# PRBonn/OverlapNet

Measured on AMD Instinct MI355X. Metric: scan-pairs/s (64x900 range images), higher is better.
Workload: dtype f32 (scaled 3-term fp16 split on the fp16 MFMA: 22 significand bits per operand, fp32 accumulate)

## Files before the change

overlapnet_amd/csrc/c3_dense.hip:

```cpp
#include "ovn_internal.h"

typedef _Float16 f16x8 __attribute__((ext_vector_type(8)));
typedef _Float16 f16x4 __attribute__((ext_vector_type(4)));

namespace {

struct ArithF16 {
  typedef _Float16 elem;
  typedef f16x8 v8;
  typedef f16x4 v4;
  static __device__ __forceinline__ f32x4 mfma(v8 a, v8 b, f32x4 c) { return __builtin_amdgcn_mfma_f32_16x16x32_f16(a, b, c, 0, 0, 0); }
};

constexpr int G = OVN_G;
constexpr int OW = OVN_O3_HW;
constexpr int CI = OVN_C2_OUT;
constexpr int CO = OVN_C3_OUT;
constexpr int NBAND = 3;
constexpr int MAX_ROWS = 8;
constexpr int MAX_MT = (MAX_ROWS * OW + 15) / 16;
constexpr int IN_PIX_MAX = (MAX_ROWS + 2) * G;
constexpr int PLANE = IN_PIX_MAX * 8 + 8;
constexpr int NPL = CI / 8;
constexpr size_t LDS_BYTES = 2 * (size_t)NPL * PLANE * sizeof(_Float16) + 64;
constexpr int NW = 8;

__device__ __forceinline__ int band_start(int b) { return b == 0 ? 0 : (b == 1 ? 8 : 15); }
__device__ __forceinline__ int band_rows(int b) { return b == 0 ? 8 : 7; }

constexpr int MT_SPLIT = 6;
template <class A, int NWV, int MSPLIT>
__global__ __launch_bounds__(64 * NWV) void c3_dense_kernel(const float* __restrict__ o2, const typename A::elem* __restrict__ wp,
                                                           const float* __restrict__ b3, const float* __restrict__ wd,
                                                           const unsigned* __restrict__ o2max, float sw3,
                                                           float* __restrict__ partial, float* __restrict__ o3,
                                                           unsigned* __restrict__ arrived, const float* __restrict__ bd,
                                                           float* __restrict__ overlap, float* __restrict__ logit) {
  typedef typename A::elem elem_t;
  typedef typename A::v8 v8_t;
  typedef typename A::v4 v4_t;
  extern __shared__ __attribute__((aligned(16))) unsigned char smem[];
  elem_t* ih = reinterpret_cast<elem_t*>(smem);
  elem_t* il = ih + NPL * PLANE;
  float* red = reinterpret_cast<float*>(il + NPL * PLANE);

  constexpr int HALVES = NW / NWV;
  constexpr int MTW = MSPLIT == 1 ? MAX_MT : MT_SPLIT;
  const int sub = blockIdx.x % (HALVES * MSPLIT);
  const int unit = blockIdx.x / (HALVES * MSPLIT), half = sub % HALVES, mh = sub / HALVES;
  const int mt0 = MT_SPLIT * mh;
  const int pair = unit / NBAND;
  const int band = unit - pair * NBAND;
  const int r0 = band_start(band);
  const int nrows = band_rows(band);
  const int npix = nrows * OW;
  const int nmt = (npix + 15) >> 4;
  const int tid = threadIdx.x;
  const int lane = tid & 63;
  const int wave_l = tid >> 6;
  const int wave = wave_l + NWV * half;
  const int lrow = lane & 15;
  const int g = lane >> 4;

  const elem_t* wsrc = wp + ((size_t)(2 * wave) * 2) * 512 + lane * 8;
  v8_t bq[3][4];
#define C3_LOAD_B(DST, KC)                                                                  \
  {                                                                                         \
    const elem_t* q = wsrc + (size_t)(KC) * (16 * 2 * 512);                                 \
    DST[0] = *reinterpret_cast<const v8_t*>(q);                                           \
    DST[1] = *reinterpret_cast<const v8_t*>(q + 512);                                     \
    DST[2] = *reinterpret_cast<const v8_t*>(q + 1024);                                    \
    DST[3] = *reinterpret_cast<const v8_t*>(q + 1536);                                    \
  }
  C3_LOAD_B(bq[0], 0)
  C3_LOAD_B(bq[1], 1)
  const float s2 = ovn_pow2_scale_for(__uint_as_float(o2max[pair]));
  const float inv = 1.0f / (s2 * sw3);
  {
    const float* src = o2 + ((long long)pair * G + r0) * G * CI;
    const int n4 = (nrows + 2) * G * CI / 4;
    constexpr int PER_THREAD = (MAX_ROWS + 2) * G * CI / 4 / (64 * NWV);
    static_assert(PER_THREAD * 64 * NWV == (MAX_ROWS + 2) * G * CI / 4, "patch does not divide over the threads");
    f32x4 v[PER_THREAD];
#pragma unroll
    for (int k = 0; k < PER_THREAD; ++k) {
      const int i = tid + k * (64 * NWV);
      v[k] = (i < n4) ? *reinterpret_cast<const f32x4*>(src + 4 * i) : (f32x4){0.f, 0.f, 0.f, 0.f};
    }
#pragma unroll
    for (int k = 0; k < PER_THREAD; ++k) {
      const int i = tid + k * (64 * NWV);
      if (i < n4) {
        const int pix = i / (CI / 4);
        const int c = 4 * (i - pix * (CI / 4));
        v4_t h, l;
#pragma unroll
        for (int e = 0; e < 4; ++e) {
          const float x = v[k][e] * s2;
          h[e] = (elem_t)x;
          l[e] = (elem_t)(x - (float)h[e]);
        }
        const int o = (c >> 3) * PLANE + pix * 8 + (c & 7);
        *reinterpret_cast<v4_t*>(ih + o) = h;
        *reinterpret_cast<v4_t*>(il + o) = l;
      }
    }
  }

  int abase[MTW];
#pragma unroll
  for (int mt = 0; mt < MTW; ++mt) {
    int p = 16 * (mt0 + mt) + lrow;
    if (p >= npix) p = npix - 1;
    const int oy = p / OW;
    const int ox = p - oy * OW;
    abase[mt] = g * PLANE + (oy * G + ox) * 8;
  }

  f32x4 acc[MTW][2];
#pragma unroll
  for (int mt = 0; mt < MTW; ++mt) {
    acc[mt][0] = (f32x4){0.f, 0.f, 0.f, 0.f};
    acc[mt][1] = (f32x4){0.f, 0.f, 0.f, 0.f};
  }

#define C3_MFMA2(M0, M1, A0H, A0L, A1H, A1L, SRC)                                                  \
  acc[M0][0] = A::mfma(A0H, SRC[0], acc[M0][0]);          \
  acc[M0][1] = A::mfma(A0H, SRC[2], acc[M0][1]);          \
  acc[M1][0] = A::mfma(A1H, SRC[0], acc[M1][0]);          \
  acc[M1][1] = A::mfma(A1H, SRC[2], acc[M1][1]);          \
  acc[M0][0] = A::mfma(A0L, SRC[0], acc[M0][0]);          \
  acc[M0][1] = A::mfma(A0L, SRC[2], acc[M0][1]);          \
  acc[M1][0] = A::mfma(A1L, SRC[0], acc[M1][0]);          \
  acc[M1][1] = A::mfma(A1L, SRC[2], acc[M1][1]);          \
  acc[M0][0] = A::mfma(A0H, SRC[1], acc[M0][0]);          \
  acc[M0][1] = A::mfma(A0H, SRC[3], acc[M0][1]);          \
  acc[M1][0] = A::mfma(A1H, SRC[1], acc[M1][0]);          \
  acc[M1][1] = A::mfma(A1H, SRC[3], acc[M1][1]);
#define C3_READ_A(BUF, SLOT, MT)                                                            \
  fh[BUF][SLOT] = *reinterpret_cast<const v8_t*>(ih + abase[MT] + toff);                  \
  fl[BUF][SLOT] = *reinterpret_cast<const v8_t*>(il + abase[MT] + toff);
#define C3_STEP(SRC, KC)                                                                    \
  {                                                                                         \
    const int tap = (KC) >> 2;                                                              \
    const int ky = tap / 3;                                                                 \
    const int toff = (ky * G + (tap - 3 * ky)) * 8 + 4 * PLANE * ((KC) & 3);                \
    v8_t fh[2][2], fl[2][2];                                                              \
    C3_READ_A(0, 0, 0)                                                                      \
    C3_READ_A(0, 1, 1)                                                                      \
    _Pragma("unroll") for (int q = 0; q < MTW / 2; ++q) {                                \
      const int cb = q & 1, nb = cb ^ 1;                                                    \
      if (q + 1 < MTW / 2) {                                                             \
        C3_READ_A(nb, 0, 2 * q + 2)                                                         \
        C3_READ_A(nb, 1, 2 * q + 3)                                                         \
      } else if (MTW % 2 == 1 && nmt == MAX_MT) {                                                           \
        C3_READ_A(nb, 0, MTW - 1)                                                        \
      }                                                                                     \
      __builtin_amdgcn_sched_barrier(0);   \
      C3_MFMA2(2 * q, 2 * q + 1, fh[cb][0], fl[cb][0], fh[cb][1], fl[cb][1], SRC)           \
      __builtin_amdgcn_sched_barrier(0);                                                    \
    }                                                                                       \
    if (MTW % 2 == 1 && nmt == MAX_MT) {                               \
      const v8_t ah = fh[(MTW / 2) & 1][0], al = fl[(MTW / 2) & 1][0];              \
      acc[MTW - 1][0] = A::mfma(ah, SRC[0], acc[MTW - 1][0]); \
      acc[MTW - 1][1] = A::mfma(ah, SRC[2], acc[MTW - 1][1]); \
      acc[MTW - 1][0] = A::mfma(al, SRC[0], acc[MTW - 1][0]); \
      acc[MTW - 1][1] = A::mfma(al, SRC[2], acc[MTW - 1][1]); \
      acc[MTW - 1][0] = A::mfma(ah, SRC[1], acc[MTW - 1][0]); \
      acc[MTW - 1][1] = A::mfma(ah, SRC[3], acc[MTW - 1][1]); \
    }                                                                                       \
  }
  __syncthreads();
#pragma unroll 1
  for (int kc = 0; kc < 36; kc += 3) {
    C3_LOAD_B(bq[2], kc + 2)
    C3_STEP(bq[0], kc)
    if (kc + 3 < 36) C3_LOAD_B(bq[0], kc + 3)
    C3_STEP(bq[1], kc + 1)
    if (kc + 4 < 36) C3_LOAD_B(bq[1], kc + 4)
    C3_STEP(bq[2], kc + 2)
  }
#undef C3_LOAD_B
#undef C3_STEP
#undef C3_MFMA2
#undef C3_READ_A

  float s[2] = {0.f, 0.f};
#pragma unroll
  for (int nt = 0; nt < 2; ++nt) {
    const int n = 32 * wave + 16 * nt + lrow;
    const float bv = b3[n];
#pragma unroll
    for (int mt = 0; mt < MTW; ++mt) {
#pragma unroll
      for (int r = 0; r < 4; ++r) {
        const int p = 16 * (mt0 + mt) + 4 * g + r;
        if (p < npix) {
          const float v = fmaxf(fmaf(acc[mt][nt][r], inv, bv), 0.0f);
          const long long fi = (long long)(r0 * OW + p) * CO + n;
          s[(MSPLIT == 1 && mt >= MT_SPLIT) ? 1 : 0] += v * wd[fi];
          if (o3) o3[(long long)pair * OVN_DENSE_IN + fi] = v;
        }
      }
    }
  }
#pragma unroll
  for (int off = 32; off > 0; off >>= 1) {
    s[0] += __shfl_down(s[0], off, 64);
    if (MSPLIT == 1) s[1] += __shfl_down(s[1], off, 64);
  }
  if (lane == 0) {
    red[wave_l] = s[0];
    if (MSPLIT == 1) red[NW + wave_l] = s[1];
  }
  __syncthreads();
  if (tid == 0) {
    float* dst = partial + ((size_t)pair * NBAND + band) * 4;
    if (NWV == NW) {
      dst[0] = (red[0] + red[1]) + (red[2] + red[3]);
      dst[1] = (red[NW + 0] + red[NW + 1]) + (red[NW + 2] + red[NW + 3]);
      dst[2] = (red[4] + red[5]) + (red[6] + red[7]);
      dst[3] = (red[NW + 4] + red[NW + 5]) + (red[NW + 6] + red[NW + 7]);
    } else {
      dst[2 * half + mh] = (red[0] + red[1]) + (red[2] + red[3]);
    }
    if (overlap != nullptr) {
      constexpr unsigned PARTS = NBAND * HALVES * MSPLIT;
      __threadfence();
      const unsigned prev = atomicAdd(arrived + pair, 1u);
      if (prev == PARTS - 1) {
        __threadfence();
        const float* q = partial + (size_t)pair * OVN_DENSE_PARTIALS;
        float z = 0.f;
#pragma unroll
        for (int b = 0; b < NBAND; ++b) {
          const float q0 = __hip_atomic_load(q + 4 * b, __ATOMIC_RELAXED, __HIP_MEMORY_SCOPE_AGENT);
          const float q1 = __hip_atomic_load(q + 4 * b + 1, __ATOMIC_RELAXED, __HIP_MEMORY_SCOPE_AGENT);
          const float q2 = __hip_atomic_load(q + 4 * b + 2, __ATOMIC_RELAXED, __HIP_MEMORY_SCOPE_AGENT);
          const float q3 = __hip_atomic_load(q + 4 * b + 3, __ATOMIC_RELAXED, __HIP_MEMORY_SCOPE_AGENT);
          const float zb = (q0 + q1) + (q2 + q3);
          z = b == 0 ? zb : z + zb;
        }
        z += bd[0];
        if (logit) logit[pair] = z;
        overlap[pair] = 1.0f / (1.0f + expf(-z));
        __hip_atomic_store(arrived + pair, 0u, __ATOMIC_RELAXED, __HIP_MEMORY_SCOPE_AGENT);
      }
    }
  }
}

__global__ __launch_bounds__(256) void dense_finish_kernel(const float* __restrict__ partial, const float* __restrict__ bd, int n,
                                                           float* __restrict__ overlap, float* __restrict__ logit) {
  const int p = blockIdx.x * 256 + threadIdx.x;
  if (p >= n) return;
  const float* q = partial + (size_t)p * OVN_DENSE_PARTIALS;
  float z = 0.f;
#pragma unroll
  for (int b = 0; b < NBAND; ++b) {
    const float zb = (q[4 * b] + q[4 * b + 1]) + (q[4 * b + 2] + q[4 * b + 3]);
    z = b == 0 ? zb : z + zb;
  }
  z += bd[0];
  if (logit) logit[p] = z;
  overlap[p] = 1.0f / (1.0f + expf(-z));
}

}

int ovn_c3_dense_forward(const ovn_ctx* ctx, const float* o2, const unsigned* o2max, int n, float* partial, float* o3,
                         unsigned* arrived, float* overlap, float* logit, hipStream_t stream) {
  OVN_REQUIRE(o2max != nullptr, OVN_ERR_ARG, "ovn_c3_dense_forward: the per-pair maxima of o2 are required");
  OVN_REQUIRE(overlap == nullptr || arrived != nullptr, OVN_ERR_ARG, "ovn_c3_dense_forward: arrival counters missing");
  int rc;
  if (n <= 21) {
    rc = ovn_allow_dynamic_lds(reinterpret_cast<const void*>(c3_dense_kernel<ArithF16, 4, 2>), LDS_BYTES);
    if (rc) return rc;
    hipLaunchKernelGGL((c3_dense_kernel<ArithF16, 4, 2>), dim3(4 * NBAND * n), dim3(64 * 4), LDS_BYTES, stream, o2,
                       reinterpret_cast<const _Float16*>(ctx->head.c3.wp_h), ctx->head.c3.bias, ctx->head.wd, o2max, ctx->head.c3.sw_h, partial, o3, arrived,
                       ctx->head.bd, overlap, logit);
  } else {
    rc = ovn_allow_dynamic_lds(reinterpret_cast<const void*>(c3_dense_kernel<ArithF16, NW, 1>), LDS_BYTES);
    if (rc) return rc;
    hipLaunchKernelGGL((c3_dense_kernel<ArithF16, NW, 1>), dim3(NBAND * n), dim3(64 * NW), LDS_BYTES, stream, o2,
                       reinterpret_cast<const _Float16*>(ctx->head.c3.wp_h), ctx->head.c3.bias, ctx->head.wd, o2max, ctx->head.c3.sw_h, partial, o3,
                       (unsigned*)nullptr, ctx->head.bd, (float*)nullptr, (float*)nullptr);
    if (overlap != nullptr)
      hipLaunchKernelGGL(dense_finish_kernel, dim3((n + 255) / 256), dim3(256), 0, stream, partial, ctx->head.bd, n, overlap, logit);
  }
  OVN_HIP_CHECK(hipGetLastError());
  return OVN_OK;
}
```

overlapnet_amd/csrc/delta_head_f16x3.hip:

```cpp
#include <math.h>
#include <stdlib.h>

#include <initializer_list>
#include <type_traits>

#include "ovn_internal.h"
#include "delta_a2.h"

typedef _Float16 f16x8 __attribute__((ext_vector_type(8)));
typedef _Float16 f16x4 __attribute__((ext_vector_type(4)));
typedef _Float16 f16x2 __attribute__((ext_vector_type(2)));
typedef __bf16 bf16x8 __attribute__((ext_vector_type(8)));

namespace {

constexpr int FW = OVN_FEAT_W;
constexpr int FC = OVN_FEAT_C;
constexpr int S = OVN_S;
constexpr int G = OVN_G;
constexpr int O1 = OVN_C1_OUT;
constexpr int O2 = OVN_C2_OUT;
constexpr int K1 = S * FC;
constexpr int K2 = S * O1;
constexpr int STEP_BYTES = 8192;
// ... 422 lines not shown
  if (packed && tid >= 64 && tid < 96) {
    const int k = tid - 64;
    if (k >= n_last) chan_s[32 * (nsl - 1) + k] = chan_s[32 * (nsl - 1) + k % n_last];
  }
  __syncthreads();
  return nlive;
}

__global__ __launch_bounds__(512) void delta_live_kernel(const float* __restrict__ feats_r, unsigned* __restrict__ live) {
  __shared__ int alive2[NPAIR][FC];
  __shared__ int neg_s;
  __shared__ int scr[2 * FC + 32];
  __shared__ __attribute__((aligned(16))) unsigned char chan_s[CHAN_BYTES];
  const int tid = threadIdx.x, c = tid & (FC - 1), part = tid >> 7;
  for (int i = tid; i < NPAIR * FC; i += 512) (&alive2[0][0])[i] = 0;
  if (tid == 0) neg_s = 0;
  __syncthreads();
  int ng = 0;
  for (int j = part; j < FW; j += 4) {
    const float v = feats_r[(size_t)j * FC + c];
    if (v != 0.0f) alive2[j / (2 * S)][c] = 1;
    ng |= (v < 0.0f);
  }
  if (ng) neg_s = 1;
  __syncthreads();
  const int nlive = build_chan_list(alive2, neg_s != 0, chan_s, scr, tid);
  store_live(live, largest_walk(chan_s), nlive, chan_s, tid);
}

__device__ __forceinline__ void w1c_gather8(const _Float16* __restrict__ w1p, const unsigned char* chan, int idx8, _Float16* __restrict__ w1c) {
  const int lane = idx8 & 63, hl = (idx8 >> 6) & 1, nt = (idx8 >> 7) & 3;
  const int step = idx8 >> 9;
  const int sc = step / S, dj = step - sc * S;
  const unsigned char* cp = chan + 32 * sc + 8 * (lane >> 4);
  const TailPack tp = tail_of(chan);
  f16x8 v;
#pragma unroll
  for (int e = 0; e < 8; ++e) {
    const int ch = cp[e];
    const int tap = (sc == tp.sl) ? tail_tap(tp, dj, 8 * (lane >> 4) + e) : dj;
    const int src_step = ((ch & 31) >> 3) * S + (tap < 0 ? 0 : tap);
    const _Float16 w = w1p[((((size_t)src_step * 4 + nt) * 2 + hl) * 64 + (lane & 15) + 16 * (ch >> 5)) * 8 + (ch & 7)];
    v[e] = tap < 0 ? (_Float16)0.0f : w;
  }
  *reinterpret_cast<f16x8*>(w1c + (size_t)idx8 * 8) = v;
}

__global__ __launch_bounds__(256) void delta_w1c_kernel(const _Float16* __restrict__ w1p, const unsigned* __restrict__ live,
                                                        _Float16* __restrict__ w1c) {
  const int ns = (int)live[0];
  const unsigned char* chan = reinterpret_cast<const unsigned char*>(live + 4);
  const int total8 = ns * S * 4 * 2 * 64;
  for (int idx8 = blockIdx.x * 256 + threadIdx.x; idx8 < total8; idx8 += gridDim.x * 256) w1c_gather8(w1p, chan, idx8, w1c);
}

__device__ __forceinline__ void glds16(const void* gsrc, void* lds_wave_base) {
  __builtin_amdgcn_global_load_lds((const __attribute__((address_space(1))) void*)gsrc,
                                   (__attribute__((address_space(3))) void*)lds_wave_base, 16, 0, 0);
}

__device__ __forceinline__ void a2_load(const float* __restrict__ a2raw, int i, float (&v)[A2_KSPLIT]) {
#pragma unroll
  for (int k = 0; k < A2_KSPLIT; ++k) v[k] = a2raw[(size_t)k * A2_ELEMS + i];
}
__device__ __forceinline__ float a2_fold(const float (&v)[A2_KSPLIT]) {
  float s = v[0];
#pragma unroll
  for (int k = 1; k < A2_KSPLIT; ++k) s += v[k];
  return s;
}
__device__ __forceinline__ void aa_product(const float* A2l, const float* __restrict__ w2sum, float* __restrict__ aa, int tid) {
  const int p = tid & (O2 - 1), jb0 = 6 * (tid >> 7);
  float wcol[O1];
#pragma unroll
  for (int o = 0; o < O1; ++o) wcol[o] = w2sum[o * O2 + p];
  float s[6] = {0.f, 0.f, 0.f, 0.f, 0.f, 0.f};
#pragma unroll
  for (int o = 0; o < O1; ++o)
#pragma unroll
    for (int j = 0; j < 6; ++j) s[j] = fmaf(A2l[(jb0 + j) * O1 + o], wcol[o], s[j]);
#pragma unroll
  for (int j = 0; j < 6; ++j) aa[(jb0 + j) * O2 + p] = s[j];
}
__device__ __forceinline__ void store_rwords8(unsigned* __restrict__ Pr, int jrow, int sc, int gq, const f32x4& v0, const f32x4& v1, float sa,
                                              float csa) {
  const int jb = jrow / S, dj = jrow - jb * S;
  unsigned* dst = Pr + ((jb * 4 + sc) * S + dj) * 32 + gq * 8;
  *reinterpret_cast<u32x4*>(dst) = pack4(v0, sa, csa);
  *reinterpret_cast<u32x4*>(dst + 4) = pack4(v1, sa, csa);
}

struct PrepWeights {
  const _Float16* wsp;
  const float* w1col;
  const float* b1;
  const _Float16* w2p;
  const float* w2sum;
  const float* b2;
  float sw1, sw2, sws, w1_colsum, b1_absmax;
};

template <bool BUILD, bool SEG = false>
__global__ __launch_bounds__(512) void delta_prepare_split_kernel(
    const float* __restrict__ feats_l, const int32_t* __restrict__ lidx, const float* __restrict__ feats_r,
    const int32_t* __restrict__ ridx, const PrepWeights W, const float* __restrict__ a2raw, float one, f32x4* __restrict__ scales,
    unsigned* __restrict__ o2max, unsigned* __restrict__ pl, unsigned* __restrict__ pr,
    float* __restrict__ lin, DeltaDesc* __restrict__ desc, const float* __restrict__ dcache, const unsigned* __restrict__ qblock,
    float* __restrict__ cache_out, const unsigned* __restrict__ live, const int32_t* __restrict__ pseg = nullptr, int seg0 = 0) {
  extern __shared__ __attribute__((aligned(16))) unsigned char psm[];
  __shared__ __attribute__((aligned(16))) unsigned char chan_p[CHAN_BYTES];
  _Float16* Th = reinterpret_cast<_Float16*>(psm);
// ... 1122 lines not shown
```

overlapnet_amd/csrc/ovn_api.hip:

```cpp
#include <stdarg.h>
#include <mutex>
#include <set>
#include <utility>
#include <stdio.h>
#include <stdlib.h>
#include <string.h>

#include <algorithm>
#include <cmath>
#include "ovn_internal.h"

int ovn_allow_dynamic_lds(const void* kernel, size_t bytes) {
  static std::mutex mu;
  static std::set<std::pair<const void*, int>> done;
  int dev = 0;
  OVN_HIP_CHECK(hipGetDevice(&dev));
  std::lock_guard<std::mutex> lock(mu);
  if (done.count({kernel, dev})) return OVN_OK;
  OVN_HIP_CHECK(hipFuncSetAttribute(kernel, hipFuncAttributeMaxDynamicSharedMemorySize, (int)bytes));
  done.insert({kernel, dev});
  return OVN_OK;
}

static thread_local char g_err[1024] = "";
// ... 117 lines not shown
    if (e != hipSuccess) {
      ovn_set_error("layer %s: keeping the raw kernel failed: %s", L->name.c_str(), hipGetErrorString(e));
      rc = OVN_ERR_HIP;
    }
  }
  if (rc) ovn_conv_release(L);
  return rc;
}

int ovn_add_leg_layer(ovn_ctx* ctx, const char* name, const float* kernel_dev, const float* bias_dev, int kh, int kw,
                      int cin, int cout, int stride_h, int stride_w, void* stream) {
  OVN_REQUIRE(ctx && name && kernel_dev && bias_dev, OVN_ERR_ARG, "ovn_add_leg_layer: NULL argument");
  OVN_REQUIRE(kh > 0 && kw > 0 && cin > 0 && cout > 0 && stride_h > 0 && stride_w > 0, OVN_ERR_ARG,
              "ovn_add_leg_layer(%s): bad geometry", name);
  OVN_REQUIRE(!ctx->finalized, OVN_ERR_STATE, "ovn_add_leg_layer(%s): context already finalized", name);
  const int expect_cin = ctx->leg.empty() ? ctx->in_c : ctx->leg.back().cout;
  OVN_REQUIRE(cin == expect_cin, OVN_ERR_ARG, "ovn_add_leg_layer(%s): cin=%d but previous layer produces %d", name, cin, expect_cin);
  OVN_ON_DEVICE(ctx->device);
  OvnConvLayer L;
  L.name = name;
  L.kh = kh;
  L.kw = kw;
  L.cin = cin;
  L.cout = cout;
  L.sh = stride_h;
  L.sw = stride_w;
  L.relu = 1;
  int rc = leg_layer_prepare(&L, kernel_dev, bias_dev, (hipStream_t)stream);
  if (rc) return rc;
  ctx->leg.push_back(L);
  return OVN_OK;
}

int ovn_set_leg_layer_weights(ovn_ctx* ctx, int layer, const float* kernel_dev, const float* bias_dev, void* stream) {
  OVN_REQUIRE(ctx && kernel_dev && bias_dev, OVN_ERR_ARG, "ovn_set_leg_layer_weights: NULL argument");
  OVN_REQUIRE(ctx->finalized, OVN_ERR_STATE, "ovn_set_leg_layer_weights: context not finalized");
  OVN_REQUIRE(layer >= 0 && layer < (int)ctx->leg.size(), OVN_ERR_ARG, "ovn_set_leg_layer_weights: no such leg layer %d", layer);
  OVN_ON_DEVICE(ctx->device);
  OvnConvLayer N = ctx->leg[layer];
  N.wp = N.bias = N.wraw = nullptr;
  N.wp_h = N.wp_h16 = nullptr;
  N.sw_h = 1.f;
  int rc = leg_layer_prepare(&N, kernel_dev, bias_dev, (hipStream_t)stream);
  if (rc) return rc;
  ovn_conv_release(&ctx->leg[layer]);
  ctx->leg[layer] = N;
  return OVN_OK;
}

void OvnHeadWeights::release() {
  ovn_conv_release(&c2);
  ovn_conv_release(&c3);
  for (void* p : {(void*)w1p, (void*)b1, w1p_h, w2p_h, (void*)w1raw, (void*)w1sum, (void*)w1col, wsp_h, (void*)w2sum, w1p_b3, w2p_b3,
                  (void*)w2raw, (void*)w3raw, (void*)wd, (void*)bd})
    if (p) (void)hipFree(p);
  *this = OvnHeadWeights();
}

static int head_keep(float** dst, const float* src, size_t n, hipStream_t stream) {
  OVN_HIP_CHECK(hipMalloc((void**)dst, n * sizeof(float)));
  OVN_HIP_CHECK(hipMemcpyAsync(*dst, src, n * sizeof(float), hipMemcpyDeviceToDevice, stream));
  return OVN_OK;
}

static OvnConvLayer head_conv(const char* name, int kh, int kw, int cin, int cout, int sh) {
  OvnConvLayer L;
  L.name = name;
  L.kh = kh;
  L.kw = kw;
  L.cin = cin;
  L.cout = cout;
  L.sh = sh;
  L.sw = 1;
  L.relu = 1;
  return L;
}

static int head_weights_prepare(OvnHeadWeights* N, int hs, int hg, const float* c1k, const float* c1b, const float* c2k, const float* c2b,
                                const float* c3k, const float* c3b, const float* dk, const float* db, hipStream_t stream) {
  const bool general = (hs != OVN_S);
  int rc = general ? head_keep(&N->w1raw, c1k, (size_t)hs * OVN_FEAT_C * OVN_C1_OUT, stream) : ovn_delta_prepare_w1(N, c1k, stream);
  if (rc == OVN_OK) rc = head_keep(&N->b1, c1b, OVN_C1_OUT, stream);
  N->c2 = head_conv("c_conv2", hs, 1, OVN_C1_OUT, OVN_C2_OUT, hs);
  if (rc == OVN_OK) rc = ovn_conv_prepare(&N->c2, c2k, c2b, stream);
  if (rc == OVN_OK && !general) rc = ovn_delta_prepare_f16x3(N, c1k, c1b, c2k, stream);
  N->c3 = head_conv("c_conv3", 3, 3, OVN_C2_OUT, OVN_C3_OUT, 1);
  if (rc == OVN_OK) rc = ovn_conv_prepare(&N->c3, c3k, c3b, stream);
  if (rc == OVN_OK && !general) rc = ovn_conv_prepare_f16x3(&N->c3, c3k, stream);
  if (rc == OVN_OK) rc = head_keep(&N->w3raw, c3k, (size_t)9 * OVN_C2_OUT * OVN_C3_OUT, stream);
  if (rc == OVN_OK && !N->w2raw) rc = head_keep(&N->w2raw, c2k, (size_t)hs * OVN_C1_OUT * OVN_C2_OUT, stream);
  if (rc == OVN_OK) rc = head_keep(&N->wd, dk, (size_t)(hg - 2) * (hg - 2) * OVN_C3_OUT, stream);
  if (rc == OVN_OK) rc = head_keep(&N->bd, db, 1, stream);
  if (rc == OVN_OK) OVN_HIP_CHECK(hipStreamSynchronize(stream));
  return rc;
}

int ovn_set_head_weights(ovn_ctx* ctx, const float* c1k, const float* c1b, const float* c2k, const float* c2b,
                         const float* c3k, const float* c3b, const float* dk, const float* db, void* stream_) {
  OVN_REQUIRE(ctx && c1k && c1b && c2k && c2b && c3k && c3b && dk && db, OVN_ERR_ARG, "ovn_set_head_weights: NULL argument");
  OVN_ON_DEVICE(ctx->device);
  const int hg = ctx_feat_w(ctx) / ctx->head_s;
  OVN_REQUIRE(hg >= 3, OVN_ERR_ARG, "ovn_set_head_weights: conv1size %d leaves %d column groups, c_conv3 needs 3", ctx->head_s, hg);
  OvnHeadWeights N;
  const int rc = head_weights_prepare(&N, ctx->head_s, hg, c1k, c1b, c2k, c2b, c3k, c3b, dk, db, (hipStream_t)stream_);
  if (rc) {
    N.release();
    return rc;
  }
  ctx->head.release();
  ctx->head = N;
  ctx->head_g = hg;
  ctx->head_set = true;
  return OVN_OK;
}

static int leg_f16x3_unserved(const ovn_ctx* ctx) {
  int h = ctx->in_h, w = ctx->in_w;
  for (size_t li = 0; li < ctx->leg.size(); ++li) {
    const auto& l = ctx->leg[li];
    if (h < l.kh || w < l.kw) return -1;
    const int oh = (h - l.kh) / l.sh + 1, ow = (w - l.kw) / l.sw + 1;
    if (li == 0 && ovn_leg_front_matches(ctx, li, h, w)) {
      const auto& l2 = ctx->leg[1];
      h = (oh - l2.kh) / l2.sh + 1;
      w = (ow - l2.kw) / l2.sw + 1;
      ++li;
      continue;
    }
    if (ovn_leg_tail_matches(ctx, li, h, w)) return -1;
    if (!ovn_conv_strip_matches(l, h, w) && (long long)oh * ow < 128) return (int)li;
    h = oh;
    w = ow;
  }
  return -1;
}

int ovn_finalize(ovn_ctx* ctx, int* feat_w) {
  OVN_REQUIRE(ctx != nullptr, OVN_ERR_ARG, "ovn_finalize: ctx is NULL");
  OVN_REQUIRE(!ctx->leg.empty(), OVN_ERR_STATE, "ovn_finalize: no leg layers registered");
  int h = ctx->in_h, w = ctx->in_w, c = ctx->in_c;
  for (const auto& l : ctx->leg) {
    OVN_REQUIRE(h >= l.kh && w >= l.kw, OVN_ERR_ARG, "ovn_finalize: layer %s does not fit its %dx%d input", l.name.c_str(), h, w);
    h = (h - l.kh) / l.sh + 1;
    w = (w - l.kw) / l.sw + 1;
// ... 1402 lines not shown
```

overlapnet_amd/csrc/ovn_internal.h:

```cpp
#pragma once

#include <hip/hip_runtime.h>
#include <math.h>
#include <stdint.h>

#include <string>
#include <vector>

#include "../../include/ovn_hip.h"
#include "ovn_scratch.h"

typedef float f32x4 __attribute__((ext_vector_type(4)));

void ovn_set_error(const char* fmt, ...);

#define OVN_HIP_CHECK(expr)                                                                   \
  do {                                                                                        \
    hipError_t _e = (expr);                                                                   \
    if (_e != hipSuccess) {                                                                   \
      ovn_set_error("%s failed: %s (%s:%d)", #expr, hipGetErrorString(_e), __FILE__, __LINE__); \
      return OVN_ERR_HIP;                                                                     \
    }                                                                                         \
  } while (0)

// ... 7 lines not shown

struct OvnDeviceGuard {
  int prev = -1;
  bool ok = false;
  explicit OvnDeviceGuard(int dev) {
    int cur = -1;
    if (hipGetDevice(&cur) != hipSuccess) return;
    if (cur == dev) {
      ok = true;
      return;
    }
    ok = (hipSetDevice(dev) == hipSuccess);
    if (ok) prev = cur;
  }
  ~OvnDeviceGuard() {
    if (prev >= 0) (void)hipSetDevice(prev);
  }
  OvnDeviceGuard(const OvnDeviceGuard&) = delete;
  OvnDeviceGuard& operator=(const OvnDeviceGuard&) = delete;
};
#define OVN_ON_DEVICE(dev)                                                             \
  OvnDeviceGuard ovn_device_guard_(dev);                                               \
  OVN_REQUIRE(ovn_device_guard_.ok, OVN_ERR_HIP, "cannot select HIP device %d", (int)(dev))

constexpr int OVN_FEAT_W = 360;
constexpr int OVN_FEAT_C = 128;
constexpr int OVN_FEAT_ELEMS = OVN_FEAT_W * OVN_FEAT_C;
constexpr int OVN_S = 15;
constexpr int OVN_G = OVN_FEAT_W / OVN_S;
constexpr int OVN_C1_OUT = 64;
constexpr int OVN_C2_OUT = 128;
constexpr int OVN_C3_OUT = 256;
constexpr int OVN_O3_HW = OVN_G - 2;
constexpr int OVN_DENSE_IN = OVN_O3_HW * OVN_O3_HW * OVN_C3_OUT;
constexpr int OVN_A2_IN_YAW_MAX_PAIRS = 64;
constexpr int OVN_DENSE_PARTIALS = 12;
constexpr int OVN_ACTMAX_SLOTS = 32;
constexpr int OVN_LEG_SLICE = 1024;
constexpr int OVN_ACTMAX_STRIDE = 32;
constexpr int OVN_SPEC_W = 368;
constexpr int OVN_SPEC_ELEMS = OVN_FEAT_C * OVN_SPEC_W;
static_assert(OVN_DELTA_CACHE_ELEMS >= OVN_FEAT_ELEMS + 24 * 128 + 4, "include/ovn_hip.h: OVN_DELTA_CACHE_ELEMS");

__host__ __device__ inline float ovn_pow2_scale_for(float m) {
  if (!(m > 0.0f) || !(m < 3.0e38f)) return 1.0f;
  int e = 0;
  (void)frexpf(m, &e);
  int k = 14 - e;
  k = k > 100 ? 100 : (k < -100 ? -100 : k);
  return ldexpf(1.0f, k);
}

#ifdef __HIPCC__
__device__ __forceinline__ void ovn_fold_absmax_wg(float vmax, unsigned* word, float* red) {
#pragma unroll
  for (int off = 32; off > 0; off >>= 1) vmax = fmaxf(vmax, __shfl_down(vmax, off, 64));
  const int nw = (blockDim.x + 63) >> 6;
  if ((threadIdx.x & 63) == 0) red[threadIdx.x >> 6] = vmax;
  __syncthreads();
  if (threadIdx.x == 0) {
    float m = red[0];
    for (int w = 1; w < nw; ++w) m = fmaxf(m, red[w]);
    const unsigned bits = __float_as_uint(m);
    if (m > 0.f && bits > __hip_atomic_load(word, __ATOMIC_RELAXED, __HIP_MEMORY_SCOPE_AGENT)) atomicMax(word, bits);
  }
}

template <int NWAVES>
__device__ __forceinline__ float ovn_wg_max_all(float m, float* red) {
#pragma unroll
  for (int off = 32; off > 0; off >>= 1) m = fmaxf(m, __shfl_down(m, off, 64));
  if ((threadIdx.x & 63) == 0) red[threadIdx.x >> 6] = m;
  __syncthreads();
  m = red[0];
#pragma unroll
  for (int w = 1; w < NWAVES; ++w) m = fmaxf(m, red[w]);
  return m;
}

template <int NWAVES>
__device__ __forceinline__ void ovn_wg_minmax_put(float mx, float mn, float* red) {
#pragma unroll
  for (int off = 32; off > 0; off >>= 1) {
    mx = fmaxf(mx, __shfl_down(mx, off, 64));
    mn = fminf(mn, __shfl_down(mn, off, 64));
  }
  if ((threadIdx.x & 63) == 0) {
    red[threadIdx.x >> 6] = mx;
    red[NWAVES + (threadIdx.x >> 6)] = mn;
  }
}
template <int NWAVES>
__device__ __forceinline__ void ovn_wg_minmax_get(const float* red, float& mx, float& mn) {
  mx = red[0];
  mn = red[NWAVES];
#pragma unroll
  for (int w = 1; w < NWAVES; ++w) {
    mx = fmaxf(mx, red[w]);
    mn = fminf(mn, red[NWAVES + w]);
  }
}

typedef _Float16 f16x8 __attribute__((ext_vector_type(8)));
typedef _Float16 f16x4 __attribute__((ext_vector_type(4)));
typedef _Float16 f16x2 __attribute__((ext_vector_type(2)));

// ... 95 lines not shown
    L.part[b][c] = ovn_norm_block_sumsq(p, b < nfull ? OVN_NORM_BLK : tail, L.m[c], a);
  }
  __syncthreads();
  if (tid < NCH) {
    double q = 0.0;
    for (int b = 0; b < nb; ++b) q += L.part[b][tid];
    L.s[tid] = 1.0 / sqrt(q > 1e-12 ? q : 1e-12);
  }
  __syncthreads();
}
#endif

struct OvnHeadScales {
  float sw1 = 1.f, sw2 = 1.f;
  float sws = 1.f;
  float w1_colsum = 0.f;
  float b1_absmax = 0.f;
};

int ovn_allow_dynamic_lds(const void* kernel, size_t bytes);

struct OvnConvLayer {
  std::string name;
  int kh = 0, kw = 0, cin = 0, cout = 0, sh = 1, sw = 1;
  int relu = 1;
  int out_cols = 0;
  int K = 0;
  int nkc = 0;
  float* wp = nullptr;
  float* bias = nullptr;
  void* wp_h = nullptr;
  float sw_h = 1.f;
  void* wp_h16 = nullptr;
  float* wraw = nullptr;
};

struct OvnHeadWeights {
  float* w1p = nullptr;
  float* b1 = nullptr;
  OvnConvLayer c2;
  OvnConvLayer c3;
  void* w1p_h = nullptr;
  void* w2p_h = nullptr;
  float* w1raw = nullptr;
  float* w1sum = nullptr;
  float* w1col = nullptr;
  void* wsp_h = nullptr;
  float* w2sum = nullptr;
  void* w1p_b3 = nullptr;
  void* w2p_b3 = nullptr;
  float* w2raw = nullptr;
  float* w3raw = nullptr;
  float* wd = nullptr;
  float* bd = nullptr;
  OvnHeadScales hs;
  void release();
};

struct ovn_ctx {
  int device = 0;
  int in_h = 0, in_w = 0, in_c = 0;
  std::vector<OvnConvLayer> leg;
  bool finalized = false;
  int feat_w = 0;
  bool head_set = false;
  int head_s = OVN_S;
  int head_g = OVN_G;
  OvnHeadWeights head;
  int leg_mode = 1;
  int head_compact = 1;
  int proj_trig = 0;
  unsigned* actmax = nullptr;
  int head_mode = 1;
  int head_width_split = 0;
  OvnConvLayer dft;
  double* tw64 = nullptr;
  int corr_norm = 0;
  float* norm_buf = nullptr;
  int64_t norm_buf_n = 0;
  void* comm = nullptr;
  int comm_rank = 0, comm_world = 1;
  int64_t head_chunk = 1024;
  int64_t head_sub = 0;
  int head_streams = 1;
  int head_yaw_side = 0;
  bool aux_ready = false;
  hipStream_t aux[2] = {nullptr, nullptr};
  hipEvent_t ev_fork = nullptr, ev_join[2] = {nullptr, nullptr};
  void* ws = nullptr;
  size_t ws_bytes = 0;
  bool prof = false;
  struct ProfRec {
    hipEvent_t a, b;
    int kind;
  };
  std::vector<ProfRec> prof_recs;
  const float* dbg_o2 = nullptr;
  const float* dbg_o3 = nullptr;
  float* dbg_partial = nullptr;
  const unsigned* dbg_o2max = nullptr;
  int64_t dbg_n = 0;
  unsigned* c3_arrived = nullptr;
  int64_t c3_arrived_n = 0;
  const unsigned* dbg_live = nullptr;
  void* seg_host = nullptr;
  void* seg_dev = nullptr;
// ... 99 lines not shown
  float *out1 = nullptr, *o2 = nullptr, *o3 = nullptr;
  OvnDeltaGenericScratch() = default;
  OvnDeltaGenericScratch(OvnCarver& c, int64_t n, int W, int G);
};
size_t ovn_delta_generic_pair_bytes(int W, int G);
int ovn_delta_generic_forward(const ovn_ctx* ctx, const float* feats_l, const int32_t* lidx, const float* feats_r,
                              const int32_t* ridx, int n, const OvnDeltaGenericScratch& scratch, float* overlap, float* logit,
                              hipStream_t stream);
int ovn_delta_generic_c1_wide(const ovn_ctx* ctx, int FW, const float* feats_l, const int32_t* lidx, const float* feats_r,
                              const int32_t* ridx, int n, float* out1, hipStream_t stream);

void ovn_head_param_sizes_of(int s, int FW, int64_t* sizes8);
int ovn_delta_head_grad_run(ovn_ctx* ctx, int FW, const float* feats_l, const int32_t* lidx, const float* feats_r, const int32_t* ridx,
                            int64_t n, const float* target, int loss, float scale, float* grad, float* loss_out, float* overlap,
                            float* o2_out, float* o3_out, hipStream_t stream,
                            float* dfeat_l = nullptr, float* dfeat_r = nullptr,
                            bool forward_only = false);

int ovn_delta_data_grad(ovn_ctx* ctx, int FW, const float* feats_l, const int32_t* lidx, const float* feats_r, const int32_t* ridx,
                        const float* dO1, int np, float* dfeat_l, float* dfeat_r, hipStream_t stream);
int ovn_yaw_grad_run(ovn_ctx* ctx, int FW, const float* feats_l, const int32_t* lidx, const float* feats_r, const int32_t* ridx,
                     int64_t n, const float* target, const int32_t* yaw_bin, float yaw_scale, float thr, float* dfeat_l, float* dfeat_r,
                     float* loss_yaw, float* corr, hipStream_t stream);

size_t ovn_leg_grad_part_bytes(const OvnConvLayer& L, int h, int w, int nb);
int ovn_leg_mask_forward(const float* dy, const float* y, float* out, long long n, hipStream_t stream);
int ovn_leg_grad_round(const double* acc, float* out, long long n, hipStream_t stream);
int ovn_leg_layer_backward(const OvnConvLayer& L, const float* x, const float* dym, int nb, int h, int w, float* dx, const float* mask,
                           double* acc_kernel, double* acc_bias, double* part, hipStream_t stream);

size_t ovn_delta_w_split_pair_bytes();
int ovn_delta_w_split_c12_forward(ovn_ctx* ctx, const float* feats_l, const int32_t* lidx, const float* feats_r, const int32_t* ridx,
                                  int n, void* scales, float* o2, hipStream_t stream);

int ovn_corr_forward(const float* feats_l, const int32_t* lidx, const float* feats_r, const int32_t* ridx, int n, int W,
                     int32_t* yaw, float* corr, hipStream_t stream, int norm_mode);

int ovn_spectral_prepare(ovn_ctx* ctx, hipStream_t stream);
int ovn_spectrum_forward(ovn_ctx* ctx, const float* feats, int n, float* spectra, hipStream_t stream);
bool ovn_conv_strip_own_scale(const OvnConvLayer& L, int h, int w);
bool ovn_conv_strip_matches(const OvnConvLayer& L, int h, int w);
int ovn_conv_strip_try(const OvnConvLayer& L, const float* in, int nb, int h, int w, float* out, const unsigned* in_max,
                       unsigned* out_max, hipStream_t stream);

bool ovn_leg_front_matches(const ovn_ctx* ctx, size_t first, int h, int w);
int ovn_leg_front_forward(const ovn_ctx* ctx, size_t first, const float* in, int nb, int h, int w, float* out, int* oh_out, int* ow_out,
                          unsigned* out_max, hipStream_t stream);

bool ovn_leg_tail_matches(const ovn_ctx* ctx, size_t first, int h, int w);
int ovn_leg_tail_forward(const ovn_ctx* ctx, size_t first, const float* in, int nb, int w, float* out, hipStream_t stream);

int ovn_c3_dense_forward(const ovn_ctx* ctx, const float* o2, const unsigned* o2max, int n, float* partial, float* o3,
                         unsigned* arrived, float* overlap, float* logit, hipStream_t stream);

int ovn_gt_range_forward(const float* points, const int64_t* offsets, int n_scans, long long max_points, const double* ref_poses,
                         const double* inv_cur_pose, int H, int W, double fov_up_deg, double fov_down_deg, double max_range,
                         float* range_out, hipStream_t stream);
int ovn_gt_count_forward(const float* ref_ranges, const float* cur_range, int n, int npix, int32_t* counts, hipStream_t stream);
int ovn_gt_pair_forward(const float* points, const int64_t* offsets, int n_scans, const double* poses, const double* inv_poses,
                        const float* cur_ranges, const int32_t* frame_idx, int n_frames, const int32_t* ref_idx, int n_refs, int H,
                        int W, double fov_up_deg, double fov_down_deg, double max_range, int frame_fastest, int32_t* counts,
                        hipStream_t stream);
int ovn_best_match_forward(const float* overlap, const int32_t* yaw, const int32_t* ids, int n, float threshold,
                           int index_offset, int32_t* out, hipStream_t stream);
int ovn_top_k_forward(const float* overlap, const int32_t* yaw, const int32_t* ids, int n, int k, float threshold,
                      int index_offset, int32_t* out, hipStream_t stream);
int ovn_top_k_segments_forward(const float* overlap, const int32_t* yaw, const int32_t* ids, const int64_t* offs_dev, int B, int k,
                               float threshold, int32_t* out, hipStream_t stream);
int ovn_segment_ridx_forward(const int64_t* offs_dev, const int32_t* qidx_dev, int B, int n, int32_t* ridx, int32_t* pseg,
                             hipStream_t stream);
int ovn_icp_register_forward(const float* vertex, const float* normal, const float* range, int n_scans, int H, int W,
                             double fov_up_deg, double fov_down_deg, double max_range, const int32_t* src_idx, const int32_t* tgt_idx,
                             int n_pairs, const double* init_pose, int iterations, double max_dist, double cos_min, double huber,
                             int min_inliers, double* pose, double* stats, double* system, hipStream_t stream);
int ovn_mcl_predict_forward(float* particles, int P, const double* motion6, uint64_t seed, uint64_t step, const int32_t* cell_frame,
                            double origin_x, double origin_y, double resolution, int nx, int ny, int M, int32_t* particle_frame,
                            int32_t* frame_slot, int32_t* frame_list, int32_t* record, hipStream_t stream);
int ovn_mcl_update_forward(float* particles, int P, const int32_t* particle_frame, const int32_t* frame_slot, const float* frame_yaw,
                           int M, const float* overlap, const int32_t* yaw, int U, double sigma_yaw, double eps_yaw, double overlap_min,
                           double* estimate, double* spread, hipStream_t stream);
int ovn_mcl_resample_forward(const float* particles, int P, uint64_t seed, uint64_t step, float* out, int n_out, int32_t* ancestor,
                             int32_t* record, hipStream_t stream);
int ovn_corr_spectral_forward(ovn_ctx* ctx, const float* spec_l, const int32_t* lidx, const float* spec_r,
                              const int32_t* ridx, int n, int32_t* yaw, float* corr, hipStream_t stream,
                              const float* a2_feats_r = nullptr, float* a2raw = nullptr);

int ovn_project_forward(ovn_ctx* ctx, const float* points, const int64_t* offsets, int n_scans,
                        int64_t max_points, int H, int W, double fov_up_deg, double fov_down_deg,
                        double max_range, float* range, float* vertex, float* intensity, int32_t* idx,
                        float* normal, float* stacked, int use_depth, int use_normals, int use_intensity,
                        hipStream_t stream);

int ovn_project_semantic_forward(ovn_ctx* ctx, const float* points, const int64_t* offsets, int n_scans, int64_t max_points, int H,
                                 int W, double fov_up_deg, double fov_down_deg, double max_range, const float* probs, int n_classes,
                                 float* range, float* vertex, float* intensity, int32_t* idx, float* normal, float* semantic,
                                 int32_t* sem_idx, float* stacked, int use_depth, int use_normals, int use_semantic, int use_intensity,
                                 hipStream_t stream);
int ovn_projection_angles_forward(const float* points, int64_t n, int H, int W, double fov_up_deg, double fov_down_deg,
                                  double max_range, float* yaw, float* pitch, int32_t* pixel, hipStream_t stream, int trig = 0);
int ovn_normals_forward(const float* range, const float* vertex, int n_scans, int H, int W, float* normal,
                        hipStream_t stream);
int ovn_normals_stack_forward(const float* range, const float* vertex, int n_scans, int H, int W, float* normal, float* stacked,
                              int use_depth, int use_normals, hipStream_t stream);

struct OvnRing {
  int base[3];
// ... 37 lines not shown
```

Before: 238,600.

## Make c3 dense kernel persistent with async prefetch of next unit's input patch

For large batches, the c3+dense kernel becomes persistent: the grid is capped at the CU count and each workgroup loops over units. While it computes the current unit, it streams the next unit's o2 patch into an extra LDS staging buffer via global_load_lds, then converts it into the fp16 hi/lo planes chunk by chunk as earlier channel chunks are consumed. The dense weights are also pre-reordered at weight-load time into accumulator order, so the epilogue reads vectorised f32x4 without per-element bounds checks. This adds LDS pressure, extra barriers per chunk and more complex control flow in exchange for hiding global-load latency and launch overhead.

```diff
diff --git a/overlapnet_amd/csrc/c3_dense.hip b/overlapnet_amd/csrc/c3_dense.hip
--- a/overlapnet_amd/csrc/c3_dense.hip
+++ b/overlapnet_amd/csrc/c3_dense.hip
@@ -24,18 +24,24 @@
 constexpr int NPL = CI / 8;
 constexpr size_t LDS_BYTES = 2 * (size_t)NPL * PLANE * sizeof(_Float16) + 64;
 constexpr int NW = 8;
+constexpr int STAGE_PIECES = IN_PIX_MAX * 8;
+constexpr size_t LDS_BYTES_RES = LDS_BYTES + (size_t)STAGE_PIECES * 16;
+static_assert(LDS_BYTES % 16 == 0 && LDS_BYTES_RES <= 160 * 1024 && STAGE_PIECES > 3 * 512 && STAGE_PIECES <= 4 * 512,
+              "staging buffer of the resident build: four rounds of 512 pieces, the last one partial");
+constexpr size_t WD_ACC_ELEMS = (size_t)NBAND * NW * 2 * MAX_MT * 64 * 4;
 
 __device__ __forceinline__ int band_start(int b) { return b == 0 ? 0 : (b == 1 ? 8 : 15); }
 __device__ __forceinline__ int band_rows(int b) { return b == 0 ? 8 : 7; }
 
 constexpr int MT_SPLIT = 6;
-template <class A, int NWV, int MSPLIT>
+template <class A, int NWV, int MSPLIT, bool RES>
 __global__ __launch_bounds__(64 * NWV) void c3_dense_kernel(const float* __restrict__ o2, const typename A::elem* __restrict__ wp,
-                                                           const float* __restrict__ b3, const float* __restrict__ wd,
+                                                           const float* __restrict__ b3, const float* __restrict__ wd_acc,
                                                            const unsigned* __restrict__ o2max, float sw3,
                                                            float* __restrict__ partial, float* __restrict__ o3,
                                                            unsigned* __restrict__ arrived, const float* __restrict__ bd,
-                                                           float* __restrict__ overlap, float* __restrict__ logit) {
+                                                           float* __restrict__ overlap, float* __restrict__ logit, int nunits) {
+  static_assert(!RES || (NWV == NW && MSPLIT == 1), "the resident build is the sweep build");
   typedef typename A::elem elem_t;
   typedef typename A::v8 v8_t;
   typedef typename A::v4 v4_t;
@@ -43,42 +49,65 @@
   elem_t* ih = reinterpret_cast<elem_t*>(smem);
   elem_t* il = ih + NPL * PLANE;
   float* red = reinterpret_cast<float*>(il + NPL * PLANE);
+  unsigned char* stage = smem + LDS_BYTES;
 
   constexpr int HALVES = NW / NWV;
   constexpr int MTW = MSPLIT == 1 ? MAX_MT : MT_SPLIT;
+  constexpr int TAP_UNROLL = RES ? 3 : 1;
   const int sub = blockIdx.x % (HALVES * MSPLIT);
-  const int unit = blockIdx.x / (HALVES * MSPLIT), half = sub % HALVES, mh = sub / HALVES;
+  const int half = sub % HALVES, mh = sub / HALVES;
   const int mt0 = MT_SPLIT * mh;
-  const int pair = unit / NBAND;
-  const int band = unit - pair * NBAND;
-  const int r0 = band_start(band);
-  const int nrows = band_rows(band);
-  const int npix = nrows * OW;
-  const int nmt = (npix + 15) >> 4;
   const int tid = threadIdx.x;
   const int lane = tid & 63;
-  const int wave_l = tid >> 6;
+  const int wave_l = __builtin_amdgcn_readfirstlane(tid >> 6);
   const int wave = wave_l + NWV * half;
   const int lrow = lane & 15;
   const int g = lane >> 4;
 
   const elem_t* wsrc = wp + ((size_t)(2 * wave) * 2) * 512 + lane * 8;
   v8_t bq[3][4];
-#define C3_LOAD_B(DST, KC)                                                                  \
+#define C3_LOAD_B(DST, S)                                                                   \
   {                                                                                         \
-    const elem_t* q = wsrc + (size_t)(KC) * (16 * 2 * 512);                                 \
+    const int ch_ = (S) / 9;                                                                \
+    const elem_t* q = wsrc + (size_t)(((S) - 9 * ch_) * 4 + ch_) * (16 * 2 * 512);          \
     DST[0] = *reinterpret_cast<const v8_t*>(q);                                           \
     DST[1] = *reinterpret_cast<const v8_t*>(q + 512);                                     \
     DST[2] = *reinterpret_cast<const v8_t*>(q + 1024);                                    \
     DST[3] = *reinterpret_cast<const v8_t*>(q + 1536);                                    \
   }
+  const int st_pix = tid >> 3, st_sub = tid & 7;
+  const int st_plane = (st_sub >> 1) * PLANE + st_pix * 8 + 4 * (st_sub & 1);
+  const unsigned st_goff = (unsigned)(st_pix * CI + 4 * st_sub) * 4u;
+#define C3_DMA_NEXT(CH)                                                                     \
+  _Pragma("unroll") for (int q = 0; q < 4; ++q)                                             \
+    if (q < 3 || wave_l < waves3_n)                                                         \
+      glds16(src_n + (size_t)((q * 64 * CI + 32 * (CH)) * 4) + (size_t)st_goff, stage + (q * 512 + wave_l * 64) * 16);
+#define C3_REFILL(TAP)                                                                      \
+  if (RES && (TAP) < 4 && fill && ((TAP) < 3 || wave_l < fill_waves3)) {                    \
+    const f32x4 v = *reinterpret_cast<const f32x4*>(stage + ((TAP) * 512 + tid) * 16);      \
+    v4_t h, l;                                                                              \
+    _Pragma("unroll") for (int e = 0; e < 4; ++e) {                                         \
+      const float x = v[e] * fill_s2;                                                       \
+      h[e] = (elem_t)x;                                                                     \
+      l[e] = (elem_t)(x - (float)h[e]);                                                     \
+    }                                                                                       \
+    const int o = st_plane + fill_plane + 512 * (TAP);                                      \
+    *reinterpret_cast<v4_t*>(ih + o) = h;                                                   \
+    *reinterpret_cast<v4_t*>(il + o) = l;                                                   \
+  }                                                                                         \
+  if (RES && (TAP) == 5) {                                                                  \
+    __builtin_amdgcn_s_waitcnt(0x0F70);    \
+    if (has_next) { C3_DMA_NEXT(chunk) }                                                    \
+  }
+  int unit = blockIdx.x / (HALVES * MSPLIT);
   C3_LOAD_B(bq[0], 0)
   C3_LOAD_B(bq[1], 1)
-  const float s2 = ovn_pow2_scale_for(__uint_as_float(o2max[pair]));
-  const float inv = 1.0f / (s2 * sw3);
+  float s2 = ovn_pow2_scale_for(__uint_as_float(o2max[unit / NBAND]));
+  bool staged = false;
   {
-    const float* src = o2 + ((long long)pair * G + r0) * G * CI;
-    const int n4 = (nrows + 2) * G * CI / 4;
+    const int pair = unit / NBAND, band = unit - pair * NBAND;
+    const float* src = o2 + ((long long)pair * G + band_start(band)) * G * CI;
+    const int n4 = (band_rows(band) + 2) * G * CI / 4;
     constexpr int PER_THREAD = (MAX_ROWS + 2) * G * CI / 4 / (64 * NWV);
     static_assert(PER_THREAD * 64 * NWV == (MAX_ROWS + 2) * G * CI / 4, "patch does not divide over the threads");
     f32x4 v[PER_THREAD];
@@ -107,6 +136,25 @@
     }
   }
 
+  do {
+  const int pair = unit / NBAND;
+  const int band = unit - pair * NBAND;
+  const int r0 = band_start(band);
+  const int npix = band_rows(band) * OW;
+  const int nmt = (npix + 15) >> 4;
+  const int waves3 = (band_rows(band) + 2) * G / 8 - 3 * NW;
+  const float inv = 1.0f / (s2 * sw3);
+  const int unit_n = unit + (int)gridDim.x;
+  const bool has_next = RES && unit_n < nunits;
+  const unsigned char* src_n = reinterpret_cast<const unsigned char*>(o2);
+  int waves3_n = 0;
+  float s2_next = 1.0f;
+  if (has_next) {
+    const int pair_n = unit_n / NBAND, band_n = unit_n - pair_n * NBAND;
+    src_n = reinterpret_cast<const unsigned char*>(o2 + ((long long)pair_n * G + band_start(band_n)) * G * CI);
+    waves3_n = (band_rows(band_n) + 2) * G / 8 - 3 * NW;
+    s2_next = ovn_pow2_scale_for(__uint_as_float(o2max[pair_n]));
+  }
   int abase[MTW];
 #pragma unroll
   for (int mt = 0; mt < MTW; ++mt) {
@@ -140,11 +188,11 @@
 #define C3_READ_A(BUF, SLOT, MT)                                                            \
   fh[BUF][SLOT] = *reinterpret_cast<const v8_t*>(ih + abase[MT] + toff);                  \
   fl[BUF][SLOT] = *reinterpret_cast<const v8_t*>(il + abase[MT] + toff);
-#define C3_STEP(SRC, KC)                                                                    \
+#define C3_STEP(SRC, CHUNK, TAP)                                                            \
   {                                                                                         \
-    const int tap = (KC) >> 2;                                                              \
-    const int ky = tap / 3;                                                                 \
-    const int toff = (ky * G + (tap - 3 * ky)) * 8 + 4 * PLANE * ((KC) & 3);                \
+    const int tp_ = (TAP);                                                                  \
+    const int ky = tp_ / 3;                                                                 \
+    const int toff = (ky * G + (tp_ - 3 * ky)) * 8 + 4 * PLANE * (CHUNK);                   \
     v8_t fh[2][2], fl[2][2];                                                              \
     C3_READ_A(0, 0, 0)                                                                      \
     C3_READ_A(0, 1, 1)                                                                      \
@@ -172,35 +220,44 @@
   }
   __syncthreads();
 #pragma unroll 1
-  for (int kc = 0; kc < 36; kc += 3) {
-    C3_LOAD_B(bq[2], kc + 2)
-    C3_STEP(bq[0], kc)
-    if (kc + 3 < 36) C3_LOAD_B(bq[0], kc + 3)
-    C3_STEP(bq[1], kc + 1)
-    if (kc + 4 < 36) C3_LOAD_B(bq[1], kc + 4)
-    C3_STEP(bq[2], kc + 2)
-  }
-#undef C3_LOAD_B
-#undef C3_STEP
-#undef C3_MFMA2
-#undef C3_READ_A
+  for (int chunk = 0; chunk < 4; ++chunk) {
+    const bool fill = RES && (chunk == 0 ? staged : has_next);
+    const float fill_s2 = chunk == 0 ? s2 : s2_next;
+    const int fill_waves3 = chunk == 0 ? waves3 : waves3_n;
+    const int fill_plane = 4 * ((chunk + 3) & 3) * PLANE;
+#pragma unroll TAP_UNROLL
+    for (int tap = 0; tap < 9; tap += 3) {
+      const int s = 9 * chunk + tap;
+      C3_LOAD_B(bq[2], s + 2)
+      C3_STEP(bq[0], chunk, tap)
+      C3_REFILL(tap)
+      if (s + 3 < 36) C3_LOAD_B(bq[0], s + 3)
+      C3_STEP(bq[1], chunk, tap + 1)
+      C3_REFILL(tap + 1)
+      if (s + 4 < 36) C3_LOAD_B(bq[1], s + 4)
+      C3_STEP(bq[2], chunk, tap + 2)
+      C3_REFILL(tap + 2)
+    }
+    if (RES && chunk < 3) __syncthreads();
+  }
 
   float s[2] = {0.f, 0.f};
+  const f32x4* wq = reinterpret_cast<const f32x4*>(wd_acc) + (size_t)(band * NW + wave) * (2 * MAX_MT * 64) + lane;
 #pragma unroll
   for (int nt = 0; nt < 2; ++nt) {
+    if (nt == 1) __builtin_amdgcn_sched_barrier(0);
     const int n = 32 * wave + 16 * nt + lrow;
     const float bv = b3[n];
 #pragma unroll
     for (int mt = 0; mt < MTW; ++mt) {
+      if (mt0 + mt >= MAX_MT) continue;
+      const f32x4 w = wq[(nt * MAX_MT + mt0 + mt) * 64];
 #pragma unroll
       for (int r = 0; r < 4; ++r) {
         const int p = 16 * (mt0 + mt) + 4 * g + r;
-        if (p < npix) {
-          const float v = fmaxf(fmaf(acc[mt][nt][r], inv, bv), 0.0f);
-          const long long fi = (long long)(r0 * OW + p) * CO + n;
-          s[(MSPLIT == 1 && mt >= MT_SPLIT) ? 1 : 0] += v * wd[fi];
-          if (o3) o3[(long long)pair * OVN_DENSE_IN + fi] = v;
-        }
+        const float v = fmaxf(fmaf(acc[mt][nt][r], inv, bv), 0.0f);
+        s[(MSPLIT == 1 && mt >= MT_SPLIT) ? 1 : 0] += v * w[r];
+        if (o3 && p < npix) o3[(long long)pair * OVN_DENSE_IN + (long long)(r0 * OW + p) * CO + n] = v;
       }
     }
   }
@@ -248,6 +305,33 @@
       }
     }
   }
+  staged = has_next;
+  if (has_next) {
+    s2 = s2_next;
+    C3_LOAD_B(bq[0], 0)
+    C3_LOAD_B(bq[1], 1)
+  }
+  unit = unit_n;
+  } while (RES && unit < nunits);
+#undef C3_LOAD_B
+#undef C3_STEP
+#undef C3_MFMA2
+#undef C3_READ_A
+#undef C3_DMA_NEXT
+#undef C3_REFILL
+}
+
+__global__ __launch_bounds__(256) void dense_acc_order_kernel(const float* __restrict__ wd, float* __restrict__ wd_acc) {
+  const int i = blockIdx.x * 256 + threadIdx.x;
+  if (i >= (int)WD_ACC_ELEMS) return;
+  const int r = i & 3, lane = (i >> 2) & 63;
+  int t = i >> 8;
+  const int mt = t % MAX_MT;
+  t /= MAX_MT;
+  const int nt = t & 1, wave = (t >> 1) % NW, band = (t >> 1) / NW;
+  const int p = 16 * mt + 4 * (lane >> 4) + r;
+  const int n = 32 * wave + 16 * nt + (lane & 15);
+  wd_acc[i] = p < band_rows(band) * OW ? wd[(size_t)(band_start(band) * OW + p) * CO + n] : 0.0f;
 }
 
 __global__ __launch_bounds__(256) void dense_finish_kernel(const float* __restrict__ partial, const float* __restrict__ bd, int n,
@@ -272,22 +356,38 @@
                          unsigned* arrived, float* overlap, float* logit, hipStream_t stream) {
   OVN_REQUIRE(o2max != nullptr, OVN_ERR_ARG, "ovn_c3_dense_forward: the per-pair maxima of o2 are required");
   OVN_REQUIRE(overlap == nullptr || arrived != nullptr, OVN_ERR_ARG, "ovn_c3_dense_forward: arrival counters missing");
+  OVN_REQUIRE(ctx->head.wd_acc != nullptr, OVN_ERR_STATE, "ovn_c3_dense_forward: no Dense kernel in accumulator order registered");
   int rc;
   if (n <= 21) {
-    rc = ovn_allow_dynamic_lds(reinterpret_cast<const void*>(c3_dense_kernel<ArithF16, 4, 2>), LDS_BYTES);
+    rc = ovn_allow_dynamic_lds(reinterpret_cast<const void*>(c3_dense_kernel<ArithF16, 4, 2, false>), LDS_BYTES);
     if (rc) return rc;
-    hipLaunchKernelGGL((c3_dense_kernel<ArithF16, 4, 2>), dim3(4 * NBAND * n), dim3(64 * 4), LDS_BYTES, stream, o2,
-                       reinterpret_cast<const _Float16*>(ctx->head.c3.wp_h), ctx->head.c3.bias, ctx->head.wd, o2max, ctx->head.c3.sw_h, partial, o3, arrived,
-                       ctx->head.bd, overlap, logit);
+    hipLaunchKernelGGL((c3_dense_kernel<ArithF16, 4, 2, false>), dim3(4 * NBAND * n), dim3(64 * 4), LDS_BYTES, stream, o2,
+                       reinterpret_cast<const _Float16*>(ctx->head.c3.wp_h), ctx->head.c3.bias, ctx->head.wd_acc, o2max, ctx->head.c3.sw_h, partial, o3, arrived,
+                       ctx->head.bd, overlap, logit, NBAND * n);
   } else {
-    rc = ovn_allow_dynamic_lds(reinterpret_cast<const void*>(c3_dense_kernel<ArithF16, NW, 1>), LDS_BYTES);
+    static int cus[64] = {};
+    const int dev = ctx->device & 63;
+    if (cus[dev] == 0) {
+      int c = 0;
+      OVN_HIP_CHECK(hipDeviceGetAttribute(&c, hipDeviceAttributeMultiprocessorCount, ctx->device));
+      cus[dev] = c > 0 ? c : 1;
+    }
+    const int grid = NBAND * n < cus[dev] ? NBAND * n : cus[dev];
+    rc = ovn_allow_dynamic_lds(reinterpret_cast<const void*>(c3_dense_kernel<ArithF16, NW, 1, true>), LDS_BYTES_RES);
     if (rc) return rc;
-    hipLaunchKernelGGL((c3_dense_kernel<ArithF16, NW, 1>), dim3(NBAND * n), dim3(64 * NW), LDS_BYTES, stream, o2,
-                       reinterpret_cast<const _Float16*>(ctx->head.c3.wp_h), ctx->head.c3.bias, ctx->head.wd, o2max, ctx->head.c3.sw_h, partial, o3,
-                       (unsigned*)nullptr, ctx->head.bd, (float*)nullptr, (float*)nullptr);
+    hipLaunchKernelGGL((c3_dense_kernel<ArithF16, NW, 1, true>), dim3(grid), dim3(64 * NW), LDS_BYTES_RES, stream, o2,
+                       reinterpret_cast<const _Float16*>(ctx->head.c3.wp_h), ctx->head.c3.bias, ctx->head.wd_acc, o2max, ctx->head.c3.sw_h, partial, o3,
+                       (unsigned*)nullptr, ctx->head.bd, (float*)nullptr, (float*)nullptr, NBAND * n);
     if (overlap != nullptr)
       hipLaunchKernelGGL(dense_finish_kernel, dim3((n + 255) / 256), dim3(256), 0, stream, partial, ctx->head.bd, n, overlap, logit);
   }
   OVN_HIP_CHECK(hipGetLastError());
   return OVN_OK;
 }
+
+int ovn_c3_dense_prepare(OvnHeadWeights* hw, hipStream_t stream) {
+  OVN_HIP_CHECK(hipMalloc((void**)&hw->wd_acc, WD_ACC_ELEMS * sizeof(float)));
+  hipLaunchKernelGGL(dense_acc_order_kernel, dim3((unsigned)((WD_ACC_ELEMS + 255) / 256)), dim3(256), 0, stream, hw->wd, hw->wd_acc);
+  OVN_HIP_CHECK(hipGetLastError());
+  return OVN_OK;
+}
diff --git a/overlapnet_amd/csrc/delta_head_f16x3.hip b/overlapnet_amd/csrc/delta_head_f16x3.hip
--- a/overlapnet_amd/csrc/delta_head_f16x3.hip
+++ b/overlapnet_amd/csrc/delta_head_f16x3.hip
@@ -498,11 +498,6 @@
   const unsigned char* chan = reinterpret_cast<const unsigned char*>(live + 4);
   const int total8 = ns * S * 4 * 2 * 64;
   for (int idx8 = blockIdx.x * 256 + threadIdx.x; idx8 < total8; idx8 += gridDim.x * 256) w1c_gather8(w1p, chan, idx8, w1c);
-}
-
-__device__ __forceinline__ void glds16(const void* gsrc, void* lds_wave_base) {
-  __builtin_amdgcn_global_load_lds((const __attribute__((address_space(1))) void*)gsrc,
-                                   (__attribute__((address_space(3))) void*)lds_wave_base, 16, 0, 0);
 }
 
 __device__ __forceinline__ void a2_load(const float* __restrict__ a2raw, int i, float (&v)[A2_KSPLIT]) {
diff --git a/overlapnet_amd/csrc/ovn_api.hip b/overlapnet_amd/csrc/ovn_api.hip
--- a/overlapnet_amd/csrc/ovn_api.hip
+++ b/overlapnet_amd/csrc/ovn_api.hip
@@ -193,7 +193,7 @@
   ovn_conv_release(&c2);
   ovn_conv_release(&c3);
   for (void* p : {(void*)w1p, (void*)b1, w1p_h, w2p_h, (void*)w1raw, (void*)w1sum, (void*)w1col, wsp_h, (void*)w2sum, w1p_b3, w2p_b3,
-                  (void*)w2raw, (void*)w3raw, (void*)wd, (void*)bd})
+                  (void*)w2raw, (void*)w3raw, (void*)wd, (void*)wd_acc, (void*)bd})
     if (p) (void)hipFree(p);
   *this = OvnHeadWeights();
 }
@@ -231,6 +231,7 @@
   if (rc == OVN_OK) rc = head_keep(&N->w3raw, c3k, (size_t)9 * OVN_C2_OUT * OVN_C3_OUT, stream);
   if (rc == OVN_OK && !N->w2raw) rc = head_keep(&N->w2raw, c2k, (size_t)hs * OVN_C1_OUT * OVN_C2_OUT, stream);
   if (rc == OVN_OK) rc = head_keep(&N->wd, dk, (size_t)(hg - 2) * (hg - 2) * OVN_C3_OUT, stream);
+  if (rc == OVN_OK && !general && hg == OVN_G) rc = ovn_c3_dense_prepare(N, stream);
   if (rc == OVN_OK) rc = head_keep(&N->bd, db, 1, stream);
   if (rc == OVN_OK) OVN_HIP_CHECK(hipStreamSynchronize(stream));
   return rc;
diff --git a/overlapnet_amd/csrc/ovn_internal.h b/overlapnet_amd/csrc/ovn_internal.h
--- a/overlapnet_amd/csrc/ovn_internal.h
+++ b/overlapnet_amd/csrc/ovn_internal.h
@@ -83,6 +83,11 @@
 }
 
 #ifdef __HIPCC__
+__device__ __forceinline__ void glds16(const void* gsrc, void* lds_wave_base) {
+  __builtin_amdgcn_global_load_lds((const __attribute__((address_space(1))) void*)gsrc,
+                                   (__attribute__((address_space(3))) void*)lds_wave_base, 16, 0, 0);
+}
+
 __device__ __forceinline__ void ovn_fold_absmax_wg(float vmax, unsigned* word, float* red) {
 #pragma unroll
   for (int off = 32; off > 0; off >>= 1) vmax = fmaxf(vmax, __shfl_down(vmax, off, 64));
@@ -284,6 +289,7 @@
   float* w2raw = nullptr;
   float* w3raw = nullptr;
   float* wd = nullptr;
+  float* wd_acc = nullptr;
   float* bd = nullptr;
   OvnHeadScales hs;
   void release();
@@ -489,6 +495,7 @@
 
 int ovn_c3_dense_forward(const ovn_ctx* ctx, const float* o2, const unsigned* o2max, int n, float* partial, float* o3,
                          unsigned* arrived, float* overlap, float* logit, hipStream_t stream);
+int ovn_c3_dense_prepare(OvnHeadWeights* hw, hipStream_t stream);
 
 int ovn_gt_range_forward(const float* points, const int64_t* offsets, int n_scans, long long max_points, const double* ref_poses,
                          const double* inv_cur_pose, int H, int W, double fov_up_deg, double fov_down_deg, double max_range,
```

After: 238,100. Within noise of the previous version (-0.2%).
